# nuclearbombmods/nbody-cosmological-simulation

Hardware: AMD Instinct MI355X
Metric: particle-steps/sec (N=65536 fp64 direct-sum leapfrog) (higher is better)
Workload: dtype f64

## Files before the change

nbody_cosmological_simulation_amd/csrc/nb_api.cpp:

```cpp
#include <algorithm>
#include <cstdlib>
#include <cstring>

#include "nb_state.h"

namespace nbhost {

std::string &last_error_string()
{
    thread_local std::string err;
    return err;
}

int fail(int code, const char *fmt, ...)
{
    char buf[512];
    va_list ap;
    va_start(ap, fmt);
    vsnprintf(buf, sizeof buf, fmt, ap);
    va_end(ap);
    last_error_string() = buf;
    return code;
}

// ... 118 lines not shown
                                            "(create a new handle for a different input dtype)");
        return NB_OK;
    }
    HIPCHK(hipSetDevice(s->cfg.device));
    s->is_f64 = f64;
    const nb_config &c = s->cfg;
    const size_t el = f64 ? 8 : 4;
    const size_t cnt = (size_t)nd(s);

    auto &sp = s->sym;
    sp.enabled = false;
    PlanInput in;
    in.n = c.n; in.dim = c.dim; in.mode = c.mode; in.flags = c.flags; in.rank = c.rank; in.nranks = c.nranks;
    in.is_f64 = s->is_f64;
    in.multi = comm_active(s);
    in.cus = device_cus(c.device);
    SymPlanHost h;
    nb_plan_sym(in, s->knobs, h);
    if (h.enabled) {
        sp.r = h.r; sp.tile_b = h.tile_b; sp.tiles = h.tiles; sp.np = h.np;
        sp.nwork = (int)h.work.size();
        sp.nslots = h.nslots;
        sp.rowsplit = h.rowsplit > 0;
    }
    const size_t pe_blocks = (size_t)((c.n + NB_BLOCK - 1) / NB_BLOCK) * s->geom.nchunks;
    s->scratch_elems = std::max<size_t>(std::max<size_t>(pe_blocks, 1024), h.enabled ? h.work.size() : 0);
    const bool prune = !f64 && grid_mode(c.mode);

    void *plan_blob = nullptr;
    const size_t plan_ints = h.enabled ? (size_t)sp.tiles * 3 : 0;
    const size_t plan_bytes = h.enabled ? arena_round(h.work.size() * sizeof(SymWork)) + arena_round(plan_ints * sizeof(int)) : 0;
    const size_t blob_bytes = plan_bytes + (prune ? arena_round(sizeof(PruneState)) : 0);
    const size_t scalars_bytes = (8 + 2 * NB_MINMAX_BLOCKS) * sizeof(double);
    std::vector<ArenaRequest> req = {
        {(void **)&s->tab, sizeof(GridTables)}, {(void **)&s->scalars, scalars_bytes}, {&s->acc, cnt * el},
        {&plan_blob, blob_bytes},
        {&s->pos, cnt * el}, {&s->vel, cnt * el}, {&s->mass, (size_t)c.n * el}, {&s->staging, cnt * 8},
        {(void **)&s->partial, (size_t)s->geom.nchunks * cnt * sizeof(double)},
        {(void **)&s->scratch, s->scratch_elems * sizeof(double)},
    };
    if (force_quant_mode(c)) req.push_back({(void **)&s->fbins, cnt * sizeof(int16_t)});
    if (prune) {
        req.push_back({(void **)&s->prune_cand, cnt * sizeof(float)});
        req.push_back({(void **)&s->prune_rho, (size_t)c.n * sizeof(float)});
        req.push_back({(void **)&s->prune_idx, (size_t)c.n * sizeof(int)});
    }
// ... 436 lines not shown
```

nbody_cosmological_simulation_amd/csrc/nb_force_sym.hip:

```cpp
#include "nb_dispatch.h"
#include "nb_force_sym_kernel.h"

namespace {


template <typename T, int D, int KICK>
__global__ void __launch_bounds__(NB_BLOCK)
pack_kernel(T *__restrict__ pos, T *__restrict__ vel, const T *__restrict__ acc, const T *__restrict__ mass,
            T *__restrict__ packed, int n, int np, T half_dt, T dt, T gfac, T pad, int p_begin, int p_end, int spread,
            T far_lim, int far_pe)
{
    const int p = p_begin + blockIdx.x * NB_BLOCK + threadIdx.x;
    if (p >= p_end) return;
    if (p < n) {
#pragma unroll
        for (int k = 0; k < D; ++k) {
            const size_t idx = (size_t)p * D + k;
            T x = pos[idx];
            if (KICK) {
                T v = vel[idx];
                if (KICK == NB_PACK_CLOSE_OPEN) v = axpy_rn<T>(v, acc[idx], half_dt);
                v = axpy_rn<T>(v, acc[idx], half_dt);
                x = axpy_rn<T>(x, v, dt);
                vel[idx] = v;
// ... 281 lines not shown
    if (p_end < 0) p_end = np;
    if (p_end <= p_begin) return hipSuccess;
    const double pad = (is_f64 && !f32_pairs) ? 1e150 : 1e18;
    const double far_lim = nb_far_limit(far, is_f64 && !f32_pairs);
    const int grid = (p_end - p_begin + NB_BLOCK - 1) / NB_BLOCK;
    const int k = (kick == NB_PACK_CLOSE_OPEN || kick == NB_PACK_OPEN) ? kick : NB_PACK_NONE;
    return nb::pick<2, 3>(dim, [&](auto D) {
        return nb::pick_real(is_f64, [&](auto real) {
            using T = typename decltype(real)::type;
            return nb::pick<NB_PACK_NONE, NB_PACK_OPEN, NB_PACK_CLOSE_OPEN>(k, [&](auto K) {
                hipLaunchKernelGGL((pack_kernel<T, D.value, K.value>), dim3(grid), dim3(NB_BLOCK), 0, st, (T *)pos, (T *)vel,
                                   (const T *)acc, (const T *)mass, (T *)packed, n, np, (T)half_dt, (T)dt, (T)gfac, (T)pad, p_begin,
                                   p_end, spread_pad, (T)far_lim, far == NB_FAR_PE ? 1 : 0);
                return hipGetLastError();
            });
        });
    });
}

hipError_t nb_launch_force_sym_f64(const double *packed, const SymWork *work, int nwork, double *rowslab,
                                   double *colslab, int np, int dim, int r, int uniform, int pa_f32, double eps2,
                                   hipStream_t st, NbKernelEvents ev, int rowsplit, int ldsrot)
{
    if (ldsrot && dim == 2 && r == 4 && !pa_f32)
        return nb::pick_bool(rowsplit, [&](auto RS) {
            if (ldsrot == SYM_ROT_DPP)
                return launch_sym_ldsrot<RS.value, SYM_ROT_DPP>(packed, work, nwork, rowslab, colslab, np, uniform, eps2, st, ev);
            return launch_sym_ldsrot<RS.value, SYM_ROT_LDS>(packed, work, nwork, rowslab, colslab, np, uniform, eps2, st, ev);
        });
    if (rowsplit) {
        if (dim != 2 || r != 4) return hipErrorInvalidValue;
        if (pa_f32) return launch_sym_rowsplit<HOOK_F32PAIR>(packed, work, nwork, rowslab, colslab, np, uniform, eps2, (float)eps2, st, ev);
        return launch_sym_rowsplit<HOOK_NONE>(packed, work, nwork, rowslab, colslab, np, uniform, eps2, 1.0f, st, ev);
    }
    return nb::pick<2, 3>(dim, [&](auto D) {
        if (pa_f32)
            return nb::pick<2, 4>(r, [&](auto R) {
                return launch_sym_u<double, D.value, R.value, HOOK_F32PAIR>(packed, work, nwork, rowslab, colslab, np, uniform, eps2,
                                                                            nullptr, (float)eps2, st, ev);
            });
        return nb::pick<1, 2, 4>(r, [&](auto R) {
            return launch_sym_u<double, D.value, R.value, HOOK_NONE>(packed, work, nwork, rowslab, colslab, np, uniform, eps2, nullptr,
                                                                     1.0f, st, ev);
        });
    });
}
// ... 75 lines not shown
```

nbody_cosmological_simulation_amd/csrc/nb_force_sym_kernel.h:

```cpp
#pragma once
#include "nb_device.h"
#include "nb_dispatch.h"
#ifdef NB_GRID_R2_EXACT
#define NB_GRID_R2_EXACT_V 1
#else
#define NB_GRID_R2_EXACT_V 0
#endif
#ifndef NB_GRID_FACTOR_LUT
#define NB_GRID_FACTOR_LUT 0
#endif
#ifndef NB_GRID_GENERAL_PACKED
#define NB_GRID_GENERAL_PACKED 2
#endif

#include <hip/hip_ext.h>

#include <type_traits>

namespace {

using namespace nbdev;

template <typename T>
__device__ __forceinline__ T rot1(T v, int addr);
// ... 72 lines not shown
        if (real) { if (exact) ++exact_pairs; else ++fast_pairs; }
    }
    __device__ __forceinline__ void rotate(int rj, int rot_addr, bool diag)
    {
        jp[rj] = __builtin_amdgcn_ds_bpermute(rot_addr, jp[rj]);
        if (!diag) {
            j1[rj] = __double_as_longlong(rot1<double>(__longlong_as_double(j1[rj]), rot_addr));
            j2[rj] = __double_as_longlong(rot1<double>(__longlong_as_double(j2[rj]), rot_addr));
        }
    }
};

typedef double d2 __attribute__((ext_vector_type(2)));
struct LdsRot {
    const d2 *ring;
    const double *ring_g;
    d2 *mail_w;
    const d2 *mail_r;
};

enum { SYM_ROT_LANES = 0,
       SYM_ROT_LDS = 1,
       SYM_ROT_DPP = 2,
       SYM_ROT_DPPALL = 3 };

constexpr int DPP_WAVE_ROL1 = 0x134;
__device__ __forceinline__ double dpp_rol1(double v)
{
    const long long b = __double_as_longlong(v);
    int lo = (int)(b & 0xffffffffll), hi = (int)(b >> 32);
    lo = __builtin_amdgcn_update_dpp(lo, lo, DPP_WAVE_ROL1, 0xf, 0xf, false);
    hi = __builtin_amdgcn_update_dpp(hi, hi, DPP_WAVE_ROL1, 0xf, 0xf, false);
    return __longlong_as_double(((long long)hi << 32) | (unsigned int)lo);
}

template <typename T, int D, int R, int RJ, bool DIAG, bool UNIFORM, int HOOK, int EST, bool BINS = false, int ROT = SYM_ROT_LANES>
__device__ __forceinline__ void sweep(const T (&xi)[R][D], const T (&gi)[R], T (&ai)[R][D], T (&xj)[RJ][D],
                                      T (&gj)[RJ], T (&aj)[RJ][D], T eps2, int rot_addr, const GridArgs &ga,
                                      int nsteps, BinDbg<R, RJ, BINS> &bd, const LdsRot lr = LdsRot{})
{
    static_assert(ROT == SYM_ROT_LANES || (std::is_same_v<T, double> && D == 2 && R == 4 && RJ == 4 && HOOK == HOOK_NONE && !BINS),
                  "LDS and DPP hand-offs: fp64, 2-D, four targets per lane, no hook, no bin read-out");
    constexpr bool LDSROT = ROT == SYM_ROT_LDS || ROT == SYM_ROT_DPP;
    T c15 = (T)1.5, c1875 = (T)1.875;
    if constexpr (std::is_same_v<T, double>) asm volatile("" : "+v"(c15), "+s"(c1875));
#pragma unroll 1
    for (int s = 0; s < nsteps; ++s) {
#pragma unroll
        for (int rj = 0; rj < RJ; ++rj) {
#pragma unroll
            for (int ri = 0; ri < R; ++ri) {
                T d[D];
                T w;
                if constexpr (std::is_same_v<T, double>) {
                    double q;
                    if (HOOK == HOOK_F32PAIR) {
                        float df[D];
#pragma unroll
                        for (int k = 0; k < D; ++k) {
                            df[k] = __fsub_rn((float)xj[rj][k], (float)xi[ri][k]);
                            d[k] = (double)df[k];
                        }
                        q = (double)r2_f32_exact<D>(df, ga.gfac);
                    } else {
#pragma unroll
// ... 231 lines not shown
#endif
                    }
                }
                const f2 wj = UNIFORM ? w : w * gj2[h];
#pragma unroll
                for (int k = 0; k < D; ++k) ai2[ri][k] = __builtin_elementwise_fma(wj, d[k], ai2[ri][k]);
                if (!DIAG) {
                    const f2 wi = UNIFORM ? w : w * gi[ri];
#pragma unroll
                    for (int k = 0; k < D; ++k) aj2[h][k] = __builtin_elementwise_fma(-wi, d[k], aj2[h][k]);
                }
            }
#pragma unroll
            for (int k = 0; k < D; ++k) {
                xj2[h][k] = rot1_f2(xj2[h][k], rot_addr);
                if (!DIAG) aj2[h][k] = rot1_f2(aj2[h][k], rot_addr);
            }
            if (!UNIFORM) gj2[h] = rot1_f2(gj2[h], rot_addr);
            if constexpr (BINS) { bd.rotate(2 * h, rot_addr, DIAG); bd.rotate(2 * h + 1, rot_addr, DIAG); }
        }
    }
}

#ifdef NB_WG_TRACE
constexpr int NB_WG_TRACE_MAX = 16384;
__device__ unsigned long long nb_wg_trace_buf[NB_WG_TRACE_MAX][8];
#endif

template <typename T, int D, int R, bool UNIFORM, int HOOK, int LPC = NB_LUT_MIN, bool BINS = false, bool RSPLIT = false,
          int ROT = SYM_ROT_LANES>
__global__ void __launch_bounds__(NB_BLOCK, BINS ? 2 : ((HOOK == HOOK_GRID && LPC > NB_LUT_MIN) || (RSPLIT && !UNIFORM) ? 3 : 4))
force_sym_kernel(const T *__restrict__ packed, const SymWork *__restrict__ work, double *__restrict__ rowslab,
                 T *__restrict__ colslab, int np, T eps2, const GridTables *__restrict__ tab, float gfac, float g_newton,
                 unsigned long long *__restrict__ bin_out, int bin_n)
{
    constexpr int B = 64 * R;
    constexpr bool F32_ = std::is_same_v<T, float>;
    constexpr int RJ = (NB_GRID_GENERAL_PACKED == 2 && F32_ && HOOK == HOOK_GRID && !UNIFORM && R == 4 && D == 2) ? 2 : sym_rj(D, R);
    constexpr int W = NB_BLOCK / 64;
    constexpr bool F32 = std::is_same_v<T, float>;
    static_assert(ROT == SYM_ROT_LANES || ROT == SYM_ROT_LDS || ROT == SYM_ROT_DPP, "hand-offs force_sym_kernel instantiates");
    constexpr bool LDSROT = ROT != SYM_ROT_LANES;
    alignas(LDSROT ? 16 : alignof(T)) __shared__ T s_aj[W][RJ][D][64];
    static_assert(!LDSROT || (!F32_ && D == 2 && R == 4 && HOOK == HOOK_NONE && !BINS), "LDS hand-off: fp64, 2-D, R = 4, no hook");
    static_assert(!LDSROT || sizeof(s_aj) == sizeof(d2) * W * RJ * 64, "the mailboxes reuse the column buffer");
    __shared__ d2 s_ring[LDSROT ? RJ : 1][LDSROT ? 128 : 1];
    __shared__ double s_ring_g[LDSROT && !UNIFORM ? RJ : 1][LDSROT && !UNIFORM ? 128 : 1];
    constexpr int lp = LPC;
    __shared__ float s_thr[HOOK == HOOK_GRID ? LPC + 1 : 1];
    __shared__ float s_lut[HOOK == HOOK_GRID ? LPC + 1 : 1];

#ifdef NB_WG_TRACE
    const unsigned long long trace_t0 = wall_clock64();
    const unsigned long long trace_c0 = __builtin_readcyclecounter();
#endif
    const SymWork wk = work[blockIdx.x];
    const int wave = RSPLIT ? __builtin_amdgcn_readfirstlane(threadIdx.x >> 6) : (int)(threadIdx.x >> 6), lane = threadIdx.x & 63;
    static_assert(!RSPLIT || (!std::is_same_v<T, float> && D == 2 && R == 4), "row-split: fp64, 2-D, four targets per lane");
    constexpr bool RS_OK = RSPLIT;
    constexpr bool rowsplit = RSPLIT;
    const int I = wk.tile_i + (rowsplit ? 0 : wave);
    const int wk_s_begin = rowsplit ? wk.s_begin + wk.s_count * wave / (NB_BLOCK / 64) : wk.s_begin;
    const int wk_s_count = rowsplit ? wk.s_begin + wk.s_count * (wave + 1) / (NB_BLOCK / 64) - wk_s_begin : wk.s_count;
    const int rot_addr = ((lane + 1) & 63) << 2;
    GridArgs ga{s_thr, s_lut, 0.0f, 0.0f, gfac, 0, lp, 0.0f, 0.0f, 0.0f, 0.0f, 0.0f};
    bool use_est = false, fast = false, degenerate = false;
    float gscale = gfac;
    int mass_exp = 0;
    if (HOOK == HOOK_GRID) {
        const int levels = tab->levels;
        fast = tab->fast_ok != 0;
        const int tm = fast ? tab->tm : 0;
        mass_exp = UNIFORM ? 0 : tm;
// ... 314 lines not shown
```

nbody_cosmological_simulation_amd/csrc/nb_plan.cpp:

```cpp
#include "nb_plan.h"

#include <algorithm>
#include <cmath>
#include <cstdlib>

namespace {
int env_int(const char *name, int dflt)
{
    const char *e = getenv(name);
    return e ? atoi(e) : dflt;
}
}

NbKnobs nb_read_knobs()
{
    NbKnobs k;
    k.sym = env_int("NB_SYM", -1);
    k.sym_r = env_int("NB_SYM_R", 0);
    k.sym_cl = std::max(0, env_int("NB_SYM_CL", 0));
    k.sym_split = env_int("NB_SYM_SPLIT", 0);
    if (k.sym_split < 1 || k.sym_split > 16) k.sym_split = 0;
    k.sym_rowsplit = env_int("NB_SYM_ROWSPLIT", -1);
    if (k.sym_rowsplit > 8) k.sym_rowsplit = -1;
    k.tail_pieces = env_int("NB_SYM_TAIL", 0);
    if (k.tail_pieces != 2 && k.tail_pieces != 4 && k.tail_pieces != 8 && k.tail_pieces != 16) k.tail_pieces = 0;
    k.sym_rot = env_int("NB_SYM_ROT", -1);
    if (k.sym_rot < 0 || k.sym_rot > 2) k.sym_rot = -1;
    k.r_onesided = env_int("NB_R", 0);
    k.no_prune = getenv("NB_NO_PRUNE") != nullptr;
    k.no_track = env_int("NB_NO_TRACK", 0) != 0;
    k.no_pe_sym = getenv("NB_NO_PE_SYM") != nullptr;
    k.no_uniform = getenv("NB_NO_UNIFORM") != nullptr;
    k.no_smalln = getenv("NB_NO_SMALLN") != nullptr;
    k.no_grid_fast = getenv("NB_NO_GRID_FAST") != nullptr;
    k.no_p2p = getenv("NB_NO_P2P") != nullptr;
    k.no_p2p_kick = getenv("NB_P2P_NO_KICK") != nullptr;
    k.no_small_fuse = getenv("NB_NO_SMALL_FUSE") != nullptr;
    k.no_spec = getenv("NB_NO_SPEC") != nullptr;
    k.no_x64 = getenv("NB_NO_X64") != nullptr;
    k.no_red_mm = getenv("NB_NO_RED_MM") != nullptr;
    k.small_max = std::max(0, env_int("NB_SMALL_MAX", 0));
    k.small_lanes = env_int("NB_SMALL_LANES", 0);
    if (k.small_lanes != 16 && k.small_lanes != 32 && k.small_lanes != 64) k.small_lanes = 0;
    return k;
}

void nb_plan_sym(const PlanInput &in, const NbKnobs &knobs, SymPlanHost &sp)
{
    sp = SymPlanHost();
    const int n = in.n, dim = in.dim, P = in.nranks;
// ... 58 lines not shown
                const double cost = rounds * ((64 + nsp - 1) / nsp + 1) * t_step[std::min<long long>(rounds, 4) - 1] +
                                    0.3 * 5.0 * (double)wgs / in.cus;
                if (cost < best) { best = cost; pieces = nsp; }
            }
            if (is_f64 && dim == 2 && cl == 1 && knobs.sym_rowsplit != 0) {
                long long rows_units = 0;
                for (int S = 0; S < SR; ++S)
                    if (ord[S] >= 0) for (int w = 0; w < 4; ++w) rows_units += std::max(0, T - (4 * S + w));
                for (int nsp : {1, 2, 3, 4}) {
                    const long long wgs = rows_units * nsp, rounds = (wgs + in.cus - 1) / in.cus;
                    const double cost = rounds * ((64 + 4 * nsp - 1) / (4 * nsp) + 1) * t_step[std::min<long long>(rounds, 4) - 1] +
                                        0.5 * 2.0 * (double)wgs / in.cus;
                    if (cost < best) { best = cost; rowsplit = nsp; }
                }
            }
        }
        for (int S = 0; S < SR; ++S) split_of[S] = pieces;
    } else if (items <= 100) {
        const int pieces = items < 24 ? 8 : (items <= 64 ? 4 : 2);
        for (int S = 0; S < SR; ++S) split_of[S] = pieces;
    } else if (sp.r == 2 && !is_f64 && items < (in.mode >= NB_INT8_SIM ? 900 : 400)) {
        for (int S = 0; S < SR; ++S) split_of[S] = 2;
    } else if (items > wg_slots / 2) {
        long long rem = items % wg_slots;
        const int pieces = knobs.tail_pieces ? knobs.tail_pieces : (sp.r == 2 ? 2 : (items < 2 * wg_slots ? 8 : 4));
        if (rem > 0 && rem <= (sp.r == 2 ? 3 * wg_slots / 8 : wg_slots / 2)) {
            for (int S = SR - 1; S >= 0 && rem > 0; --S)
                if (ord[S] >= 0) { split_of[S] = pieces; rem -= nch_of[S]; }
        }
    }

    if (knobs.sym_rowsplit > 0 && is_f64 && dim == 2 && sp.r == 4 && in.mode == NB_FLOAT64) rowsplit = knobs.sym_rowsplit;
    if (in.mode != NB_FLOAT64) rowsplit = 0;

    std::vector<SymWork> items_v;
    int slots = 0, ncol = 0;
    if (rowsplit > 0) {
        const int nsp = rowsplit;
        sp.col_upto.assign(sp.tiles, 0);
        for (int I = 0; I < sp.tiles; ++I) {
            sp.col_upto[I] = ncol;
            sp.row_slot0[I] = slots;
            sp.row_nslots[I] = 0;
            if (I >= T || ord[I >> 2] < 0) continue;
            const int nch = (T - I + cl - 1) / cl;
            sp.row_nslots[I] = nch * nsp;
// ... 46 lines not shown
```

nbody_cosmological_simulation_amd/csrc/nb_plan.h:

```cpp
#pragma once
#include <vector>

#include "nb_internal.h"

#ifndef NB_SYM_ROT_DEFAULT
#define NB_SYM_ROT_DEFAULT 2
#endif

struct NbKnobs {
    int sym = -1;
    int sym_r = 0;
    int sym_cl = 0;
    int sym_split = 0;
    int sym_rowsplit = -1;
    int tail_pieces = 0;
    int sym_rot = -1;
    int r_onesided = 0;
    bool no_prune = false;
    bool no_track = false;
    bool no_pe_sym = false;
    bool no_uniform = false;
    bool no_smalln = false;
    int small_max = 0;
    int small_lanes = 0;
    bool no_grid_fast = false;
    bool no_p2p = false;
    bool no_red_mm = false;
    bool no_x64 = false;
    bool no_small_fuse = false;
    bool no_p2p_kick = false;
    bool no_spec = false;
};
NbKnobs nb_read_knobs();

struct SymPlanHost {
    bool enabled = false;
    int r = 2, tile_b = 128, tiles = 0, np = 0, nslots = 0, ncol = 0, cl = 1;
    int rowsplit = 0;
    std::vector<SymWork> work;
    std::vector<int> row_slot0, row_nslots, col_upto;
    size_t col_bytes = 0, row_bytes = 0, packed_bytes = 0;
};

struct PlanInput {
    int n = 0, dim = 2, mode = 0, flags = 0, rank = 0, nranks = 1;
    bool is_f64 = true;
    bool multi = false;
    int cus = 256;
};

void nb_plan_sym(const PlanInput &in, const NbKnobs &knobs, SymPlanHost &out);
```

nbody_cosmological_simulation_amd/csrc/nb_state.h:

```cpp
#pragma once
#include <rccl/rccl.h>

#include <cmath>
#include <cstdarg>
#include <cstdint>
#include <cstdio>
#include <mutex>
#include <string>
#include <vector>

#include "nb_internal.h"
#include "nb_plan.h"

namespace nbhost {

std::string &last_error_string();
int fail(int code, const char *fmt, ...);

#define HIPCHK(expr)                                                                              \
    do {                                                                                          \
        hipError_t e_ = (expr);                                                                   \
        if (e_ != hipSuccess)                                                                     \
            return ::nbhost::fail(e_ == hipErrorOutOfMemory ? NB_ERR_OOM : NB_ERR_HIP, "%s failed: %s (%s:%d)", #expr, \
                                  hipGetErrorString(e_), __FILE__, __LINE__);                     \
// ... 66 lines not shown
    void *pos = nullptr, *vel = nullptr, *mass = nullptr, *acc = nullptr;
    double *partial = nullptr;
    void *staging = nullptr;
    GridTables *tab = nullptr;
    double *scratch = nullptr;
    size_t scratch_elems = 0;
    double *scalars = nullptr;
    int16_t *fbins = nullptr;
    float *prune_cand = nullptr, *prune_rho = nullptr;
    int *prune_idx = nullptr;
    PruneState *prune_state = nullptr;
    bool prune_seeded = false;
    bool mass_uniform = false;
    double mass_value = 0.0;
    const char *last_kernel = "none";
    char pe_kernel[96] = "none";
    std::string path_part[3];
    std::string step_path = "none";
    bool path_open_kd = false;
    ForceGeom geom{};
    struct SymPlan {
        bool enabled = false;
        bool rowsplit = false;
        int r = 2, tile_b = 128, tiles = 0, np = 0, nwork = 0, nslots = 0;
        SymWork *work = nullptr;
        int *row_slot0 = nullptr, *row_nslots = nullptr, *col_upto = nullptr;
        void *packed = nullptr, *colslab = nullptr;
        double *rowslab = nullptr;
    } sym;
    void *pos_alt = nullptr;
    bool spec_open = false;
    double spec_dt = 0.0;
    int spec_kind = 0;
    double *small_part = nullptr;
    void *gen_scalars = nullptr;
    bool last_generic = false;
    bool used_p2p = false;
    double *sums64 = nullptr;
    void *metrics_scratch = nullptr;
    size_t metrics_cap = 0;
    unsigned long long *bin_out = nullptr;
    NbKnobs knobs;
    ncclComm_t comm = nullptr;
    unsigned comm_generation = 0;
    hipEvent_t ev_start[nbhost::PROF_RING], ev_stop[nbhost::PROF_RING];
    bool prof_init = false;
// ... 73 lines not shown
```

nbody_cosmological_simulation_amd/csrc/nb_step.cpp:

```cpp
#include <algorithm>
#include <cstring>

#include "nb_state.h"

namespace nbhost {

struct NbTuning {
    int onesided_r1_max_n = 8192;
    int onesided_target_wgs = 1024;
    int prune_min_n = 8192;
    int track_min_n = 3072;
    int red_mm_max_blocks = 1024;
    int small_max_f64 = 4096;
    int small_max_f32 = 3072;
    int small_fuse_tables_max_n = 2048;
};
static const NbTuning g_tune{};

int small_max_n(bool is_f64) { return is_f64 ? g_tune.small_max_f64 : g_tune.small_max_f32; }

int onesided_r(int n, const NbKnobs &knobs)
{
    if (knobs.r_onesided == 1 || knobs.r_onesided == 2 || knobs.r_onesided == 4)
        return knobs.r_onesided;
// ... 263 lines not shown
    unsigned long long *bin_out = (rq.bins && grid) ? s->bin_out : nullptr;
    int slot;
    if (!e.used_sym) {
        if (int rc = prof_begin(s, &slot)) return rc;
        if (s->is_f64)
            HIPCHK(nb_launch_force_f64((const double *)s->pos, (const double *)s->mass, s->partial, s->geom, c.dim, e.pair_dt,
                                       e.hook, c.G, c.softening_sq, e.eps2, s->stream));
        else
            HIPCHK(nb_launch_force_f32((const float *)s->pos, (const float *)s->mass, s->partial, s->geom, c.dim, e.hook,
                                       e.pair_dt, (float)c.G, e.eps2, s->tab, L, s->stream, bin_out));
        s->last_kernel = s->is_f64 ? "force_f64_kernel" : "force_f32_kernel";
        return prof_end(s, slot);
    }
    const int pa_f32 = s->is_f64 && e.pair_dt == NB_F32;
    if (!rq.packed_ready) {
        const double gfac = s->is_f64 ? c.G : (grid ? 1.0 : (double)(float)c.G);
        HIPCHK(nb_launch_pack(s->pos, s->vel, s->acc, s->mass, sp.packed, c.n, sp.np, c.dim, s->is_f64, NB_PACK_NONE, 0.0, 0.0,
                              gfac, pa_f32, s->stream, 0, -1, 0, grid ? NB_FAR_OFF : NB_FAR_FORCE));
    }
    if (int rc = prof_begin(s, &slot, false)) return rc;
    if (s->is_f64) {
        HIPCHK(nb_launch_force_sym_f64((const double *)sp.packed, sp.work, sp.nwork, sp.rowslab, (double *)sp.colslab, sp.np,
                                       c.dim, sp.r, s->mass_uniform, pa_f32, c.softening_sq, s->stream, prof_events(s, slot),
                                       sp.rowsplit ? 1 : 0, s->knobs.sym_rot >= 0 ? s->knobs.sym_rot : NB_SYM_ROT_DEFAULT));
        s->last_kernel = "force_sym_kernel<double";
        return NB_OK;
    }
    const bool uniform = grid ? (s->mass_uniform && sp.r != 2) : e.sym_uniform;
    if (bin_out)
        HIPCHK(nb_launch_force_sym_f32_bins((const float *)sp.packed, sp.work, sp.nwork, sp.rowslab, (float *)sp.colslab, sp.np,
                                            c.dim, sp.r, uniform, e.eps2, s->tab, (float)c.G, (float)s->mass_value, L, bin_out,
                                            c.n, s->stream));
    else
        HIPCHK(nb_launch_force_sym_f32((const float *)sp.packed, sp.work, sp.nwork, sp.rowslab, (float *)sp.colslab, sp.np,
                                       c.dim, sp.r, uniform, e.hook, e.eps2, s->tab, (float)c.G, (float)s->mass_value, L,
                                       s->stream, prof_events(s, slot)));
    s->last_kernel = "force_sym_kernel<float";
    return NB_OK;
}

int reduce_and_exchange(nb_sim *s, const EvalRequest &rq, Eval &e, EvalResult *res)
{
    const nb_config &c = s->cfg;
    const int64_t cnt = nd(s);
    const bool p2p = e.multi && (e.x64 ? p2p_use_x64(s, cnt) : p2p_use(s, cnt));
    void *red_out = p2p ? nb_p2p_data() : (rq.bins ? s->staging : s->acc);
    if (e.x64 && !p2p && !s->sums64) HIPCHK(hipMalloc((void **)&s->sums64, (size_t)cnt * sizeof(double)));
// ... 378 lines not shown
```

Measured before the change: 57.77 million.

## Add eight-target DPP ring sweep for whole-sweep fp64 symmetric force

Adds a new hand-off mode in which each lane holds eight target particles, covering two tile pairs, instead of four. It sweeps a shared LDS source ring with DPP rotation of the column accumulators, and the four waves split into tile pairs and step halves whose row partials are combined through LDS at the end. The planner marks large single-rank runs (n >= 32768) as whole sweeps and selects this mode by default for them. The aim is to raise arithmetic per source load and per DPP rotation. The cost is higher register pressure and extra block-wide syncs per source tile.

```diff
diff --git a/nbody_cosmological_simulation_amd/csrc/nb_api.cpp b/nbody_cosmological_simulation_amd/csrc/nb_api.cpp
--- a/nbody_cosmological_simulation_amd/csrc/nb_api.cpp
+++ b/nbody_cosmological_simulation_amd/csrc/nb_api.cpp
@@ -164,6 +164,7 @@
         sp.nwork = (int)h.work.size();
         sp.nslots = h.nslots;
         sp.rowsplit = h.rowsplit > 0;
+        sp.rot = s->knobs.sym_rot >= 0 ? s->knobs.sym_rot : (h.whole_sweeps ? NB_SYM_ROT_WHOLE_DEFAULT : NB_SYM_ROT_DEFAULT);
     }
     const size_t pe_blocks = (size_t)((c.n + NB_BLOCK - 1) / NB_BLOCK) * s->geom.nchunks;
     s->scratch_elems = std::max<size_t>(std::max<size_t>(pe_blocks, 1024), h.enabled ? h.work.size() : 0);
diff --git a/nbody_cosmological_simulation_amd/csrc/nb_force_sym.hip b/nbody_cosmological_simulation_amd/csrc/nb_force_sym.hip
--- a/nbody_cosmological_simulation_amd/csrc/nb_force_sym.hip
+++ b/nbody_cosmological_simulation_amd/csrc/nb_force_sym.hip
@@ -327,6 +327,9 @@
                                    double *colslab, int np, int dim, int r, int uniform, int pa_f32, double eps2,
                                    hipStream_t st, NbKernelEvents ev, int rowsplit, int ldsrot)
 {
+    if (ldsrot == SYM_ROT_DPP8 && dim == 2 && r == 4 && !pa_f32 && !rowsplit)
+        return launch_sym_ldsrot<false, SYM_ROT_DPP8>(packed, work, nwork, rowslab, colslab, np, uniform, eps2, st, ev);
+    if (ldsrot == SYM_ROT_DPP8) ldsrot = SYM_ROT_DPP;
     if (ldsrot && dim == 2 && r == 4 && !pa_f32)
         return nb::pick_bool(rowsplit, [&](auto RS) {
             if (ldsrot == SYM_ROT_DPP)
diff --git a/nbody_cosmological_simulation_amd/csrc/nb_force_sym_kernel.h b/nbody_cosmological_simulation_amd/csrc/nb_force_sym_kernel.h
--- a/nbody_cosmological_simulation_amd/csrc/nb_force_sym_kernel.h
+++ b/nbody_cosmological_simulation_amd/csrc/nb_force_sym_kernel.h
@@ -118,7 +118,8 @@
 enum { SYM_ROT_LANES = 0,
        SYM_ROT_LDS = 1,
        SYM_ROT_DPP = 2,
-       SYM_ROT_DPPALL = 3 };
+       SYM_ROT_DPP8 = 3,
+       SYM_ROT_DPPALL = 4 };
 
 constexpr int DPP_WAVE_ROL1 = 0x134;
 __device__ __forceinline__ double dpp_rol1(double v)
@@ -135,8 +136,9 @@
                                       T (&gj)[RJ], T (&aj)[RJ][D], T eps2, int rot_addr, const GridArgs &ga,
                                       int nsteps, BinDbg<R, RJ, BINS> &bd, const LdsRot lr = LdsRot{})
 {
-    static_assert(ROT == SYM_ROT_LANES || (std::is_same_v<T, double> && D == 2 && R == 4 && RJ == 4 && HOOK == HOOK_NONE && !BINS),
-                  "LDS and DPP hand-offs: fp64, 2-D, four targets per lane, no hook, no bin read-out");
+    static_assert(ROT == SYM_ROT_LANES || (std::is_same_v<T, double> && D == 2 && HOOK == HOOK_NONE && !BINS &&
+                                           ((R == 4 && RJ == 4) || ((R == 4 || R == 8) && (RJ == 2 || RJ == 4) && ROT != SYM_ROT_DPPALL))),
+                  "LDS and DPP hand-offs: fp64, 2-D, four targets per lane (ring modes: four or eight, against two or four source slots), no hook, no bin read-out");
     constexpr bool LDSROT = ROT == SYM_ROT_LDS || ROT == SYM_ROT_DPP;
     T c15 = (T)1.5, c1875 = (T)1.875;
     if constexpr (std::is_same_v<T, double>) asm volatile("" : "+v"(c15), "+s"(c1875));
@@ -414,6 +416,137 @@
     }
 }
 
+#ifndef NB_SYM_DPP8_RJ
+#define NB_SYM_DPP8_RJ 2
+#endif
+
+template <bool UNIFORM, int RJ8>
+__device__ __forceinline__ void force_sym_dpp8(const double *__restrict__ packed, const SymWork &wk, double *__restrict__ rowslab,
+                                               double *__restrict__ colslab, int np, double eps2, double *s_aj, d2 *s_ring,
+                                               double *s_ring_g)
+{
+    constexpr int D = 2, R = 4, R8 = 8, B = 64 * R, W = NB_BLOCK / 64;
+    static_assert(W == 4 && (RJ8 == 2 || RJ8 == 4), "two tile pairs x two step halves; the source tile whole or in two halves");
+    const int wave = __builtin_amdgcn_readfirstlane(threadIdx.x >> 6), lane = threadIdx.x & 63;
+    const int pr = wave & 1, hf = wave >> 1;
+    const int I0 = wk.tile_i + 2 * pr;
+    const int s_begin = wk.s_begin + wk.s_count * hf / 2;
+    const int s_count = wk.s_begin + wk.s_count * (hf + 1) / 2 - s_begin;
+    const GridArgs ga{};
+    BinDbg<R8, RJ8, false> bd8;
+    BinDbg<R, RJ8, false> bd4;
+
+    double xi[R8][D], gi[R8], ai[R8][D];
+#pragma unroll
+    for (int r = 0; r < R8; ++r) {
+        const int p = I0 * B + r * 64 + lane;
+#pragma unroll
+        for (int k = 0; k < D; ++k) {
+            xi[r][k] = packed[(size_t)k * np + p];
+            ai[r][k] = 0.0;
+        }
+        gi[r] = UNIFORM ? 1.0 : packed[(size_t)D * np + p];
+    }
+
+    auto thread_index = [wave] {
+        int l;
+        asm volatile("v_mbcnt_lo_u32_b32 %0, -1, 0\n\tv_mbcnt_hi_u32_b32 %0, -1, %0" : "=v"(l));
+        return wave * 64 + l;
+    };
+    auto stage_ring = [&](int Jt, int tid) {
+        const int e = (tid >> 6) * 128 + (tid & 63);
+        const size_t p = (size_t)Jt * B + tid;
+        const d2 v = {packed[p], packed[(size_t)np + p]};
+        s_ring[e] = v;
+        s_ring[e + 64] = v;
+        if constexpr (!UNIFORM) {
+            const double g = packed[(size_t)D * np + p];
+            s_ring_g[e] = g;
+            s_ring_g[e + 64] = g;
+        }
+    };
+    if (wk.jt_begin < wk.jt_end) stage_ring(wk.jt_begin, threadIdx.x);
+    __syncthreads();
+
+    auto load_sources = [&](const LdsRot &lh, double (&xj)[RJ8][D], double (&gj)[RJ8]) {
+#pragma unroll
+        for (int r = 0; r < RJ8; ++r) {
+            const d2 x0 = lh.ring[r * 128];
+            xj[r][0] = x0.x;
+            xj[r][1] = x0.y;
+            if constexpr (UNIFORM) gj[r] = 1.0;
+            else gj[r] = lh.ring_g[r * 128];
+        }
+    };
+    auto sweep4 = [&](auto t, auto diag, const LdsRot &lh, double (&aj)[RJ8][D]) {
+        constexpr int T0 = decltype(t)::value * R;
+        double xj[RJ8][D], gj[RJ8];
+        load_sources(lh, xj, gj);
+        sweep<double, D, R, RJ8, decltype(diag)::value, UNIFORM, HOOK_NONE, 0, false, SYM_ROT_DPP>(
+            reinterpret_cast<const double (&)[R][D]>(xi[T0]), reinterpret_cast<const double (&)[R]>(gi[T0]),
+            reinterpret_cast<double (&)[R][D]>(ai[T0]), xj, gj, aj, eps2, 0, ga, s_count, bd4, lh);
+    };
+
+    for (int J = wk.jt_begin; J < wk.jt_end; ++J) {
+#pragma unroll
+        for (int half = 0; half < R / RJ8; ++half) {
+            const int hs = half * RJ8;
+            const int e0 = hs * 128 + (thread_index() & 63) + s_begin;
+            const LdsRot lh{s_ring + e0, UNIFORM ? s_ring_g : s_ring_g + e0, nullptr, nullptr};
+            double aj[RJ8][D];
+#pragma unroll
+            for (int r = 0; r < RJ8; ++r) aj[r][0] = aj[r][1] = 0.0;
+            if (J > I0 + 1) {
+                double xj[RJ8][D], gj[RJ8];
+                load_sources(lh, xj, gj);
+                sweep<double, D, R8, RJ8, false, UNIFORM, HOOK_NONE, 0, false, SYM_ROT_DPP>(xi, gi, ai, xj, gj, aj, eps2, 0, ga, s_count,
+                                                                                           bd8, lh);
+            } else if (J == I0 + 1) {
+                sweep4(std::integral_constant<int, 1>{}, std::true_type{}, lh, aj);
+                sweep4(std::integral_constant<int, 0>{}, std::false_type{}, lh, aj);
+            } else if (J == I0) {
+                sweep4(std::integral_constant<int, 0>{}, std::true_type{}, lh, aj);
+            }
+            double *const col = s_aj + (size_t)wave * (R * D * 64) + ((thread_index() + s_begin + s_count) & 63);
+#pragma unroll
+            for (int r = 0; r < RJ8; ++r)
+#pragma unroll
+                for (int k = 0; k < D; ++k) col[((hs + r) * D + k) * 64] = aj[r][k];
+        }
+        __syncthreads();
+        const int tid = thread_index();
+        if (J + 1 < wk.jt_end) stage_ring(J + 1, tid);
+        if (J > wk.tile_i) {
+            for (int idx = tid; idx < R * D * 64; idx += NB_BLOCK) {
+                const int l = idx & 63, rk = idx >> 6;
+                double v = s_aj[rk * 64 + l];
+#pragma unroll
+                for (int w = 1; w < W; ++w) v += s_aj[(w * R * D + rk) * 64 + l];
+                colslab[((size_t)wk.col_ord * D + (rk % D)) * np + (size_t)J * B + (rk / D) * 64 + l] = v;
+            }
+        }
+        __syncthreads();
+    }
+
+    const int ln = thread_index() & 63;
+    if (hf == 1) {
+#pragma unroll
+        for (int r = 0; r < R8; ++r)
+#pragma unroll
+            for (int k = 0; k < D; ++k) s_aj[((pr * R8 + r) * D + k) * 64 + ln] = ai[r][k];
+    }
+    __syncthreads();
+    if (hf == 0) {
+#pragma unroll
+        for (int r = 0; r < R8; ++r) {
+            const int slot = wk.slot + (2 * pr + r / R) * wk.slot_stride;
+#pragma unroll
+            for (int k = 0; k < D; ++k)
+                rowslab[((size_t)slot * D + k) * B + (r % R) * 64 + ln] = ai[r][k] + s_aj[((pr * R8 + r) * D + k) * 64 + ln];
+        }
+    }
+}
+
 #ifdef NB_WG_TRACE
 constexpr int NB_WG_TRACE_MAX = 16384;
 __device__ unsigned long long nb_wg_trace_buf[NB_WG_TRACE_MAX][8];
@@ -431,7 +564,8 @@
     constexpr int RJ = (NB_GRID_GENERAL_PACKED == 2 && F32_ && HOOK == HOOK_GRID && !UNIFORM && R == 4 && D == 2) ? 2 : sym_rj(D, R);
     constexpr int W = NB_BLOCK / 64;
     constexpr bool F32 = std::is_same_v<T, float>;
-    static_assert(ROT == SYM_ROT_LANES || ROT == SYM_ROT_LDS || ROT == SYM_ROT_DPP, "hand-offs force_sym_kernel instantiates");
+    static_assert(ROT == SYM_ROT_LANES || ROT == SYM_ROT_LDS || ROT == SYM_ROT_DPP || ROT == SYM_ROT_DPP8,
+                  "hand-offs force_sym_kernel instantiates");
     constexpr bool LDSROT = ROT != SYM_ROT_LANES;
     alignas(LDSROT ? 16 : alignof(T)) __shared__ T s_aj[W][RJ][D][64];
     static_assert(!LDSROT || (!F32_ && D == 2 && R == 4 && HOOK == HOOK_NONE && !BINS), "LDS hand-off: fp64, 2-D, R = 4, no hook");
@@ -441,6 +575,13 @@
     constexpr int lp = LPC;
     __shared__ float s_thr[HOOK == HOOK_GRID ? LPC + 1 : 1];
     __shared__ float s_lut[HOOK == HOOK_GRID ? LPC + 1 : 1];
+
+    if constexpr (ROT == SYM_ROT_DPP8) {
+        static_assert(ROT != SYM_ROT_DPP8 || (!RSPLIT && sizeof(s_aj) == sizeof(double) * 2 * 16 * 64), "classic work items only");
+        force_sym_dpp8<UNIFORM, NB_SYM_DPP8_RJ>(packed, work[blockIdx.x], rowslab, colslab, np, eps2, &s_aj[0][0][0][0],
+                                                      &s_ring[0][0], &s_ring_g[0][0]);
+        return;
+    }
 
 #ifdef NB_WG_TRACE
     const unsigned long long trace_t0 = wall_clock64();
diff --git a/nbody_cosmological_simulation_amd/csrc/nb_plan.cpp b/nbody_cosmological_simulation_amd/csrc/nb_plan.cpp
--- a/nbody_cosmological_simulation_amd/csrc/nb_plan.cpp
+++ b/nbody_cosmological_simulation_amd/csrc/nb_plan.cpp
@@ -25,7 +25,7 @@
     k.tail_pieces = env_int("NB_SYM_TAIL", 0);
     if (k.tail_pieces != 2 && k.tail_pieces != 4 && k.tail_pieces != 8 && k.tail_pieces != 16) k.tail_pieces = 0;
     k.sym_rot = env_int("NB_SYM_ROT", -1);
-    if (k.sym_rot < 0 || k.sym_rot > 2) k.sym_rot = -1;
+    if (k.sym_rot < 0 || k.sym_rot > 3) k.sym_rot = -1;
     k.r_onesided = env_int("NB_R", 0);
     k.no_prune = getenv("NB_NO_PRUNE") != nullptr;
     k.no_track = env_int("NB_NO_TRACK", 0) != 0;
@@ -130,6 +130,7 @@
     } else if (sp.r == 2 && !is_f64 && items < (in.mode >= NB_INT8_SIM ? 900 : 400)) {
         for (int S = 0; S < SR; ++S) split_of[S] = 2;
     } else if (items > wg_slots / 2) {
+        sp.whole_sweeps = P == 1 && n >= NB_SYM_ROT_WHOLE_FROM;
         long long rem = items % wg_slots;
         const int pieces = knobs.tail_pieces ? knobs.tail_pieces : (sp.r == 2 ? 2 : (items < 2 * wg_slots ? 8 : 4));
         if (rem > 0 && rem <= (sp.r == 2 ? 3 * wg_slots / 8 : wg_slots / 2)) {
diff --git a/nbody_cosmological_simulation_amd/csrc/nb_plan.h b/nbody_cosmological_simulation_amd/csrc/nb_plan.h
--- a/nbody_cosmological_simulation_amd/csrc/nb_plan.h
+++ b/nbody_cosmological_simulation_amd/csrc/nb_plan.h
@@ -5,6 +5,12 @@
 
 #ifndef NB_SYM_ROT_DEFAULT
 #define NB_SYM_ROT_DEFAULT 2
+#endif
+#ifndef NB_SYM_ROT_WHOLE_DEFAULT
+#define NB_SYM_ROT_WHOLE_DEFAULT 3
+#endif
+#ifndef NB_SYM_ROT_WHOLE_FROM
+#define NB_SYM_ROT_WHOLE_FROM 32768
 #endif
 
 struct NbKnobs {
@@ -37,6 +43,7 @@
     bool enabled = false;
     int r = 2, tile_b = 128, tiles = 0, np = 0, nslots = 0, ncol = 0, cl = 1;
     int rowsplit = 0;
+    bool whole_sweeps = false;
     std::vector<SymWork> work;
     std::vector<int> row_slot0, row_nslots, col_upto;
     size_t col_bytes = 0, row_bytes = 0, packed_bytes = 0;
diff --git a/nbody_cosmological_simulation_amd/csrc/nb_state.h b/nbody_cosmological_simulation_amd/csrc/nb_state.h
--- a/nbody_cosmological_simulation_amd/csrc/nb_state.h
+++ b/nbody_cosmological_simulation_amd/csrc/nb_state.h
@@ -112,6 +112,7 @@
     struct SymPlan {
         bool enabled = false;
         bool rowsplit = false;
+        int rot = 0;
         int r = 2, tile_b = 128, tiles = 0, np = 0, nwork = 0, nslots = 0;
         SymWork *work = nullptr;
         int *row_slot0 = nullptr, *row_nslots = nullptr, *col_upto = nullptr;
diff --git a/nbody_cosmological_simulation_amd/csrc/nb_step.cpp b/nbody_cosmological_simulation_amd/csrc/nb_step.cpp
--- a/nbody_cosmological_simulation_amd/csrc/nb_step.cpp
+++ b/nbody_cosmological_simulation_amd/csrc/nb_step.cpp
@@ -309,7 +309,7 @@
     if (s->is_f64) {
         HIPCHK(nb_launch_force_sym_f64((const double *)sp.packed, sp.work, sp.nwork, sp.rowslab, (double *)sp.colslab, sp.np,
                                        c.dim, sp.r, s->mass_uniform, pa_f32, c.softening_sq, s->stream, prof_events(s, slot),
-                                       sp.rowsplit ? 1 : 0, s->knobs.sym_rot >= 0 ? s->knobs.sym_rot : NB_SYM_ROT_DEFAULT));
+                                       sp.rowsplit ? 1 : 0, sp.rot));
         s->last_kernel = "force_sym_kernel<double";
         return NB_OK;
     }
diff --git a/profiles/r8_inner_loop.s b/profiles/r8_inner_loop.s
--- /dev/null
+++ b/profiles/r8_inner_loop.s
@@ -0,0 +1,268 @@
+.LBB13_24:
+	s_waitcnt lgkmcnt(1)
+	v_add_f64 v[80:81], v[2:3], -v[16:17]
+	v_add_f64 v[78:79], v[0:1], -v[8:9]
+	v_fma_f64 v[82:83], v[80:81], v[80:81], s[12:13]
+	v_fmac_f64_e32 v[82:83], v[78:79], v[78:79]
+	v_rsq_f64_e32 v[84:85], v[82:83]
+	s_add_i32 s17, s17, -1
+	s_cmp_eq_u32 s17, 0
+	v_mul_f64 v[86:87], v[84:85], v[84:85]
+	v_fma_f64 v[82:83], -v[82:83], v[86:87], 1.0
+	v_mul_f64 v[84:85], v[84:85], v[86:87]
+	v_fma_f64 v[86:87], s[24:25], v[82:83], v[76:77]
+	v_mul_f64 v[82:83], v[82:83], v[86:87]
+	v_fmac_f64_e32 v[84:85], v[84:85], v[82:83]
+	v_fmac_f64_e32 v[70:71], v[84:85], v[78:79]
+	v_fmac_f64_e32 v[72:73], v[84:85], v[80:81]
+	v_fma_f64 v[78:79], -v[84:85], v[78:79], v[108:109]
+	v_fma_f64 v[80:81], -v[84:85], v[80:81], v[110:111]
+	v_add_f64 v[84:85], v[2:3], -v[18:19]
+	v_add_f64 v[82:83], v[0:1], -v[10:11]
+	v_fma_f64 v[86:87], v[84:85], v[84:85], s[12:13]
+	v_fmac_f64_e32 v[86:87], v[82:83], v[82:83]
+	v_rsq_f64_e32 v[88:89], v[86:87]
+	s_nop 0
+	v_mul_f64 v[90:91], v[88:89], v[88:89]
+	v_fma_f64 v[86:87], -v[86:87], v[90:91], 1.0
+	v_mul_f64 v[88:89], v[88:89], v[90:91]
+	v_fma_f64 v[90:91], s[24:25], v[86:87], v[76:77]
+	v_mul_f64 v[86:87], v[86:87], v[90:91]
+	v_fmac_f64_e32 v[88:89], v[88:89], v[86:87]
+	v_fmac_f64_e32 v[68:69], v[88:89], v[84:85]
+	v_fma_f64 v[80:81], -v[88:89], v[84:85], v[80:81]
+	v_add_f64 v[84:85], v[2:3], -v[20:21]
+	v_fmac_f64_e32 v[74:75], v[88:89], v[82:83]
+	v_fma_f64 v[78:79], -v[88:89], v[82:83], v[78:79]
+	v_add_f64 v[82:83], v[0:1], -v[12:13]
+	v_fma_f64 v[86:87], v[84:85], v[84:85], s[12:13]
+	v_fmac_f64_e32 v[86:87], v[82:83], v[82:83]
+	v_rsq_f64_e32 v[88:89], v[86:87]
+	s_nop 0
+	v_mul_f64 v[90:91], v[88:89], v[88:89]
+	v_fma_f64 v[86:87], -v[86:87], v[90:91], 1.0
+	v_mul_f64 v[88:89], v[88:89], v[90:91]
+	v_fma_f64 v[90:91], s[24:25], v[86:87], v[76:77]
+	v_mul_f64 v[86:87], v[86:87], v[90:91]
+	v_fmac_f64_e32 v[88:89], v[88:89], v[86:87]
+	v_fmac_f64_e32 v[62:63], v[88:89], v[84:85]
+	v_fma_f64 v[80:81], -v[88:89], v[84:85], v[80:81]
+	v_add_f64 v[84:85], v[2:3], -v[22:23]
+	v_fmac_f64_e32 v[54:55], v[88:89], v[82:83]
+	v_fma_f64 v[78:79], -v[88:89], v[82:83], v[78:79]
+	v_add_f64 v[82:83], v[0:1], -v[14:15]
+	v_fma_f64 v[86:87], v[84:85], v[84:85], s[12:13]
+	v_fmac_f64_e32 v[86:87], v[82:83], v[82:83]
+	v_rsq_f64_e32 v[88:89], v[86:87]
+	s_nop 0
+	v_mul_f64 v[90:91], v[88:89], v[88:89]
+	v_fma_f64 v[86:87], -v[86:87], v[90:91], 1.0
+	v_mul_f64 v[88:89], v[88:89], v[90:91]
+	v_fma_f64 v[90:91], s[24:25], v[86:87], v[76:77]
+	v_mul_f64 v[86:87], v[86:87], v[90:91]
+	v_fmac_f64_e32 v[88:89], v[88:89], v[86:87]
+	v_fmac_f64_e32 v[66:67], v[88:89], v[84:85]
+	v_fma_f64 v[80:81], -v[88:89], v[84:85], v[80:81]
+	v_add_f64 v[84:85], v[2:3], -v[26:27]
+	v_fmac_f64_e32 v[64:65], v[88:89], v[82:83]
+	v_fma_f64 v[78:79], -v[88:89], v[82:83], v[78:79]
+	v_add_f64 v[82:83], v[0:1], -v[24:25]
+	v_fma_f64 v[86:87], v[84:85], v[84:85], s[12:13]
+	v_fmac_f64_e32 v[86:87], v[82:83], v[82:83]
+	v_rsq_f64_e32 v[88:89], v[86:87]
+	s_nop 0
+	v_mul_f64 v[90:91], v[88:89], v[88:89]
+	v_fma_f64 v[86:87], -v[86:87], v[90:91], 1.0
+	v_mul_f64 v[88:89], v[88:89], v[90:91]
+	v_fma_f64 v[90:91], s[24:25], v[86:87], v[76:77]
+	v_mul_f64 v[86:87], v[86:87], v[90:91]
+	v_fmac_f64_e32 v[88:89], v[88:89], v[86:87]
+	v_fmac_f64_e32 v[58:59], v[88:89], v[84:85]
+	v_fma_f64 v[80:81], -v[88:89], v[84:85], v[80:81]
+	v_add_f64 v[84:85], v[2:3], -v[30:31]
+	v_fmac_f64_e32 v[60:61], v[88:89], v[82:83]
+	v_fma_f64 v[78:79], -v[88:89], v[82:83], v[78:79]
+	v_add_f64 v[82:83], v[0:1], -v[28:29]
+	v_fma_f64 v[86:87], v[84:85], v[84:85], s[12:13]
+	v_fmac_f64_e32 v[86:87], v[82:83], v[82:83]
+	v_rsq_f64_e32 v[88:89], v[86:87]
+	s_nop 0
+	v_mul_f64 v[90:91], v[88:89], v[88:89]
+	v_fma_f64 v[86:87], -v[86:87], v[90:91], 1.0
+	v_mul_f64 v[88:89], v[88:89], v[90:91]
+	v_fma_f64 v[90:91], s[24:25], v[86:87], v[76:77]
+	v_mul_f64 v[86:87], v[86:87], v[90:91]
+	v_fmac_f64_e32 v[88:89], v[88:89], v[86:87]
+	v_fmac_f64_e32 v[52:53], v[88:89], v[84:85]
+	v_fma_f64 v[80:81], -v[88:89], v[84:85], v[80:81]
+	v_add_f64 v[84:85], v[2:3], -v[34:35]
+	v_fmac_f64_e32 v[56:57], v[88:89], v[82:83]
+	v_fma_f64 v[78:79], -v[88:89], v[82:83], v[78:79]
+	v_add_f64 v[82:83], v[0:1], -v[32:33]
+	v_fma_f64 v[86:87], v[84:85], v[84:85], s[12:13]
+	v_fmac_f64_e32 v[86:87], v[82:83], v[82:83]
+	v_rsq_f64_e32 v[88:89], v[86:87]
+	v_add_f64 v[2:3], v[2:3], -v[38:39]
+	v_add_f64 v[0:1], v[0:1], -v[36:37]
+	v_mul_f64 v[90:91], v[88:89], v[88:89]
+	v_fma_f64 v[86:87], -v[86:87], v[90:91], 1.0
+	v_mul_f64 v[88:89], v[88:89], v[90:91]
+	v_fma_f64 v[90:91], s[24:25], v[86:87], v[76:77]
+	v_mul_f64 v[86:87], v[86:87], v[90:91]
+	v_fmac_f64_e32 v[88:89], v[88:89], v[86:87]
+	v_fmac_f64_e32 v[50:51], v[88:89], v[82:83]
+	v_fma_f64 v[78:79], -v[88:89], v[82:83], v[78:79]
+	v_fma_f64 v[82:83], v[2:3], v[2:3], s[12:13]
+	v_fmac_f64_e32 v[82:83], v[0:1], v[0:1]
+	v_fmac_f64_e32 v[48:49], v[88:89], v[84:85]
+	v_fma_f64 v[80:81], -v[88:89], v[84:85], v[80:81]
+	v_rsq_f64_e32 v[84:85], v[82:83]
+	s_nop 0
+	v_mul_f64 v[86:87], v[84:85], v[84:85]
+	v_fma_f64 v[82:83], -v[82:83], v[86:87], 1.0
+	v_mul_f64 v[84:85], v[84:85], v[86:87]
+	v_fma_f64 v[86:87], s[24:25], v[82:83], v[76:77]
+	v_mul_f64 v[82:83], v[82:83], v[86:87]
+	v_fmac_f64_e32 v[84:85], v[84:85], v[82:83]
+	v_fma_f64 v[110:111], -v[84:85], v[2:3], v[80:81]
+	s_waitcnt lgkmcnt(0)
+	v_add_f64 v[80:81], v[6:7], -v[16:17]
+	v_fma_f64 v[108:109], -v[84:85], v[0:1], v[78:79]
+	v_add_f64 v[78:79], v[4:5], -v[8:9]
+	v_fma_f64 v[82:83], v[80:81], v[80:81], s[12:13]
+	v_fmac_f64_e32 v[82:83], v[78:79], v[78:79]
+	v_fmac_f64_e32 v[46:47], v[84:85], v[0:1]
+	v_fmac_f64_e32 v[44:45], v[84:85], v[2:3]
+	v_rsq_f64_e32 v[84:85], v[82:83]
+	ds_read_b128 v[0:3], v40
+	v_mov_b32_dpp v108, v108 wave_rol:1 row_mask:0xf bank_mask:0xf
+	v_mov_b32_dpp v109, v109 wave_rol:1 row_mask:0xf bank_mask:0xf
+	v_mul_f64 v[86:87], v[84:85], v[84:85]
+	v_fma_f64 v[82:83], -v[82:83], v[86:87], 1.0
+	v_mul_f64 v[84:85], v[84:85], v[86:87]
+	v_fma_f64 v[86:87], s[24:25], v[82:83], v[76:77]
+	v_mul_f64 v[82:83], v[82:83], v[86:87]
+	v_fmac_f64_e32 v[84:85], v[84:85], v[82:83]
+	v_fmac_f64_e32 v[70:71], v[84:85], v[78:79]
+	v_fmac_f64_e32 v[72:73], v[84:85], v[80:81]
+	v_fma_f64 v[78:79], -v[84:85], v[78:79], v[114:115]
+	v_fma_f64 v[80:81], -v[84:85], v[80:81], v[112:113]
+	v_add_f64 v[84:85], v[6:7], -v[18:19]
+	v_add_f64 v[82:83], v[4:5], -v[10:11]
+	v_fma_f64 v[86:87], v[84:85], v[84:85], s[12:13]
+	v_fmac_f64_e32 v[86:87], v[82:83], v[82:83]
+	v_rsq_f64_e32 v[88:89], v[86:87]
+	v_mov_b32_dpp v110, v110 wave_rol:1 row_mask:0xf bank_mask:0xf
+	v_mov_b32_dpp v111, v111 wave_rol:1 row_mask:0xf bank_mask:0xf
+	v_mul_f64 v[90:91], v[88:89], v[88:89]
+	v_fma_f64 v[86:87], -v[86:87], v[90:91], 1.0
+	v_mul_f64 v[88:89], v[88:89], v[90:91]
+	v_fma_f64 v[90:91], s[24:25], v[86:87], v[76:77]
+	v_mul_f64 v[86:87], v[86:87], v[90:91]
+	v_fmac_f64_e32 v[88:89], v[88:89], v[86:87]
+	v_fmac_f64_e32 v[68:69], v[88:89], v[84:85]
+	v_fma_f64 v[80:81], -v[88:89], v[84:85], v[80:81]
+	v_add_f64 v[84:85], v[6:7], -v[20:21]
+	v_fmac_f64_e32 v[74:75], v[88:89], v[82:83]
+	v_fma_f64 v[78:79], -v[88:89], v[82:83], v[78:79]
+	v_add_f64 v[82:83], v[4:5], -v[12:13]
+	v_fma_f64 v[86:87], v[84:85], v[84:85], s[12:13]
+	v_fmac_f64_e32 v[86:87], v[82:83], v[82:83]
+	v_rsq_f64_e32 v[88:89], v[86:87]
+	s_nop 0
+	v_mul_f64 v[90:91], v[88:89], v[88:89]
+	v_fma_f64 v[86:87], -v[86:87], v[90:91], 1.0
+	v_mul_f64 v[88:89], v[88:89], v[90:91]
+	v_fma_f64 v[90:91], s[24:25], v[86:87], v[76:77]
+	v_mul_f64 v[86:87], v[86:87], v[90:91]
+	v_fmac_f64_e32 v[88:89], v[88:89], v[86:87]
+	v_fmac_f64_e32 v[62:63], v[88:89], v[84:85]
+	v_fma_f64 v[80:81], -v[88:89], v[84:85], v[80:81]
+	v_add_f64 v[84:85], v[6:7], -v[22:23]
+	v_fmac_f64_e32 v[54:55], v[88:89], v[82:83]
+	v_fma_f64 v[78:79], -v[88:89], v[82:83], v[78:79]
+	v_add_f64 v[82:83], v[4:5], -v[14:15]
+	v_fma_f64 v[86:87], v[84:85], v[84:85], s[12:13]
+	v_fmac_f64_e32 v[86:87], v[82:83], v[82:83]
+	v_rsq_f64_e32 v[88:89], v[86:87]
+	s_nop 0
+	v_mul_f64 v[90:91], v[88:89], v[88:89]
+	v_fma_f64 v[86:87], -v[86:87], v[90:91], 1.0
+	v_mul_f64 v[88:89], v[88:89], v[90:91]
+	v_fma_f64 v[90:91], s[24:25], v[86:87], v[76:77]
+	v_mul_f64 v[86:87], v[86:87], v[90:91]
+	v_fmac_f64_e32 v[88:89], v[88:89], v[86:87]
+	v_fmac_f64_e32 v[66:67], v[88:89], v[84:85]
+	v_fma_f64 v[80:81], -v[88:89], v[84:85], v[80:81]
+	v_add_f64 v[84:85], v[6:7], -v[26:27]
+	v_fmac_f64_e32 v[64:65], v[88:89], v[82:83]
+	v_fma_f64 v[78:79], -v[88:89], v[82:83], v[78:79]
+	v_add_f64 v[82:83], v[4:5], -v[24:25]
+	v_fma_f64 v[86:87], v[84:85], v[84:85], s[12:13]
+	v_fmac_f64_e32 v[86:87], v[82:83], v[82:83]
+	v_rsq_f64_e32 v[88:89], v[86:87]
+	s_nop 0
+	v_mul_f64 v[90:91], v[88:89], v[88:89]
+	v_fma_f64 v[86:87], -v[86:87], v[90:91], 1.0
+	v_mul_f64 v[88:89], v[88:89], v[90:91]
+	v_fma_f64 v[90:91], s[24:25], v[86:87], v[76:77]
+	v_mul_f64 v[86:87], v[86:87], v[90:91]
+	v_fmac_f64_e32 v[88:89], v[88:89], v[86:87]
+	v_fmac_f64_e32 v[58:59], v[88:89], v[84:85]
+	v_fma_f64 v[80:81], -v[88:89], v[84:85], v[80:81]
+	v_add_f64 v[84:85], v[6:7], -v[30:31]
+	v_fmac_f64_e32 v[60:61], v[88:89], v[82:83]
+	v_fma_f64 v[78:79], -v[88:89], v[82:83], v[78:79]
+	v_add_f64 v[82:83], v[4:5], -v[28:29]
+	v_fma_f64 v[86:87], v[84:85], v[84:85], s[12:13]
+	v_fmac_f64_e32 v[86:87], v[82:83], v[82:83]
+	v_rsq_f64_e32 v[88:89], v[86:87]
+	s_nop 0
+	v_mul_f64 v[90:91], v[88:89], v[88:89]
+	v_fma_f64 v[86:87], -v[86:87], v[90:91], 1.0
+	v_mul_f64 v[88:89], v[88:89], v[90:91]
+	v_fma_f64 v[90:91], s[24:25], v[86:87], v[76:77]
+	v_mul_f64 v[86:87], v[86:87], v[90:91]
+	v_fmac_f64_e32 v[88:89], v[88:89], v[86:87]
+	v_fmac_f64_e32 v[52:53], v[88:89], v[84:85]
+	v_fma_f64 v[80:81], -v[88:89], v[84:85], v[80:81]
+	v_add_f64 v[84:85], v[6:7], -v[34:35]
+	v_fmac_f64_e32 v[56:57], v[88:89], v[82:83]
+	v_fma_f64 v[78:79], -v[88:89], v[82:83], v[78:79]
+	v_add_f64 v[82:83], v[4:5], -v[32:33]
+	v_fma_f64 v[86:87], v[84:85], v[84:85], s[12:13]
+	v_fmac_f64_e32 v[86:87], v[82:83], v[82:83]
+	v_rsq_f64_e32 v[88:89], v[86:87]
+	v_add_f64 v[6:7], v[6:7], -v[38:39]
+	v_add_f64 v[4:5], v[4:5], -v[36:37]
+	v_mul_f64 v[90:91], v[88:89], v[88:89]
+	v_fma_f64 v[86:87], -v[86:87], v[90:91], 1.0
+	v_mul_f64 v[88:89], v[88:89], v[90:91]
+	v_fma_f64 v[90:91], s[24:25], v[86:87], v[76:77]
+	v_mul_f64 v[86:87], v[86:87], v[90:91]
+	v_fmac_f64_e32 v[88:89], v[88:89], v[86:87]
+	v_fmac_f64_e32 v[50:51], v[88:89], v[82:83]
+	v_fma_f64 v[78:79], -v[88:89], v[82:83], v[78:79]
+	v_fma_f64 v[82:83], v[6:7], v[6:7], s[12:13]
+	v_fmac_f64_e32 v[82:83], v[4:5], v[4:5]
+	v_fmac_f64_e32 v[48:49], v[88:89], v[84:85]
+	v_fma_f64 v[80:81], -v[88:89], v[84:85], v[80:81]
+	v_rsq_f64_e32 v[84:85], v[82:83]
+	s_nop 0
+	v_mul_f64 v[86:87], v[84:85], v[84:85]
+	v_fma_f64 v[82:83], -v[82:83], v[86:87], 1.0
+	v_mul_f64 v[84:85], v[84:85], v[86:87]
+	v_fma_f64 v[86:87], s[24:25], v[82:83], v[76:77]
+	v_mul_f64 v[82:83], v[82:83], v[86:87]
+	v_fmac_f64_e32 v[84:85], v[84:85], v[82:83]
+	v_fmac_f64_e32 v[46:47], v[84:85], v[4:5]
+	v_fmac_f64_e32 v[44:45], v[84:85], v[6:7]
+	v_fma_f64 v[114:115], -v[84:85], v[4:5], v[78:79]
+	v_fma_f64 v[112:113], -v[84:85], v[6:7], v[80:81]
+	ds_read_b128 v[4:7], v40 offset:2048
+	v_mov_b32_dpp v114, v114 wave_rol:1 row_mask:0xf bank_mask:0xf
+	v_mov_b32_dpp v115, v115 wave_rol:1 row_mask:0xf bank_mask:0xf
+	v_mov_b32_dpp v112, v112 wave_rol:1 row_mask:0xf bank_mask:0xf
+	v_mov_b32_dpp v113, v113 wave_rol:1 row_mask:0xf bank_mask:0xf
+	v_add_u32_e32 v40, 16, v40
+	s_cbranch_scc0 .LBB13_24
```

Result: no change. 58.27 million (median of 6 runs) (+0.9%).
